# OpenVVC/VVCSoftware_VTM

Measured on AMD Instinct MI355X. Metric: encoded frames/sec (bit-exact bitstream) at 4K10 RA QP32, 1/2/4/8 GPU [M1: hot-path pictures/s of the kernels behind the call sites, NOT EncoderApp fps], higher is better.
Workload: dtype int16

## Files before the change

### vvcsoftware_vtm_amd/csrc/alf.hip

```cpp
#include "common.h"
#include <cstddef>

namespace {

constexpr int CT = 64;
constexpr int CP = 72;
constexpr int CR = CT + 6;
constexpr int QN = CT / 4 + 1;

template <int PITCH>
__device__ __forceinline__ void load_tile_clamped(short* __restrict__ lds, const Pel* __restrict__ src,
                                                  int stride, int w, int h, int x0, int y0, int rows,
                                                  int tid, int nthreads)
{
  constexpr int VPR = PITCH / 4;
  const int nvec = rows * VPR;
  const bool vec_ok = ((stride & 3) == 0) && ((reinterpret_cast<uintptr_t>(src) & 7) == 0);
  for (int v = tid; v < nvec; v += nthreads)
  {
    const int r = v / VPR, c = (v - r * VPR) * 4;
    int y = y0 + r;
    y = y < 0 ? 0 : (y >= h ? h - 1 : y);
    const int x = x0 + c;
    const Pel* row = src + (size_t)y * stride;
    pel4 val;
    if (vec_ok && x >= 0 && x + 3 < w)
      val = *reinterpret_cast<const pel4*>(row + x);
    else
    {
#pragma unroll
      for (int k = 0; k < 4; k++)
      {
        int xx = x + k;
        xx = xx < 0 ? 0 : (xx >= w ? w - 1 : xx);
        val[k] = row[xx];
      }
    }
    *reinterpret_cast<pel4*>(lds + r * PITCH + c) = val;
  }
}

__global__ __launch_bounds__(320) void alf_classify_kernel(const Pel* __restrict__ src, int stride, int w, int h,
                                                           int shift, uint16_t* __restrict__ cls, int gx, int total, int xcd)
{
  __shared__ short tile[CR * CP];
  __shared__ int quad[QN * QN * 4];
  const int tid = threadIdx.x;
  const int b = vvc_xcd_index((int)blockIdx.x, total, xcd);
  if (b < 0) return;
  const int by = b / gx, bx = b - by * gx;
  const int tx0 = bx * CT, ty0 = by * CT;
  load_tile_clamped<CP>(tile, src, stride, w, h, tx0 - 4, ty0 - 3, CR, tid, 320);
  __syncthreads();

  if (tid < QN * QN)
  {
    const int qi = tid / QN, qj = tid - qi * QN;
    const unsigned* base = reinterpret_cast<const unsigned*>(tile + (4 * qi) * CP + 4 * qj);
    unsigned sv = 0, sh = 0, sd0 = 0, sd1 = 0;
    unsigned A[5], B[5], C[5];
    auto loadRow = [&](int r, unsigned (&P)[5])
    {
      const uint2 lo = *reinterpret_cast<const uint2*>(base + r * (CP / 2)), hi = *reinterpret_cast<const uint2*>(base + r * (CP / 2) + 2);
      P[0] = __builtin_amdgcn_alignbit(lo.y, lo.x, 16); P[1] = lo.y; P[2] = __builtin_amdgcn_alignbit(hi.x, lo.y, 16); P[3] = hi.x;
      P[4] = __builtin_amdgcn_alignbit(hi.y, hi.x, 16);
    };
    typedef unsigned short us2v __attribute__((ext_vector_type(2)));
    auto padd = [](unsigned a, unsigned b) { return __builtin_bit_cast(unsigned, __builtin_bit_cast(us2v, a) + __builtin_bit_cast(us2v, b)); };
    loadRow(0, A); loadRow(1, B);
#pragma unroll
    for (int y = 0; y < 4; y++)
    {
      loadRow(y + 2, C);
      const unsigned c01 = padd(B[1], B[1]), c23 = padd(B[3], B[3]);
      sv  = __builtin_amdgcn_sad_u16(c01, padd(A[1], C[1]), sv);   sv  = __builtin_amdgcn_sad_u16(c23, padd(A[3], C[3]), sv);
      sh  = __builtin_amdgcn_sad_u16(c01, padd(B[0], B[2]), sh);   sh  = __builtin_amdgcn_sad_u16(c23, padd(B[2], B[4]), sh);
      sd0 = __builtin_amdgcn_sad_u16(c01, padd(A[0], C[2]), sd0);  sd0 = __builtin_amdgcn_sad_u16(c23, padd(A[2], C[4]), sd0);
      sd1 = __builtin_amdgcn_sad_u16(c01, padd(C[0], A[2]), sd1);  sd1 = __builtin_amdgcn_sad_u16(c23, padd(C[2], A[4]), sd1);
#pragma unroll
      for (int k = 0; k < 5; k++) { A[k] = B[k]; B[k] = C[k]; }
    }
    int* q = quad + tid * 4;
    q[0] = (int)sv; q[1] = (int)sh; q[2] = (int)sd0; q[3] = (int)sd1;
  }
  __syncthreads();

  if (tid < 256)
  {
    const int bi = tid >> 4, bj = tid & 15;
    const int by = ty0 + 4 * bi, bx = tx0 + 4 * bj;
    if (by < h && bx < w)
    {
      const int* q00 = quad + (bi * QN + bj) * 4;
      const int* q01 = q00 + 4;
      const int* q10 = q00 + QN * 4;
      const int* q11 = q10 + 4;
      const int sumV = q00[0] + q01[0] + q10[0] + q11[0];
      const int sumH = q00[1] + q01[1] + q10[1] + q11[1];
      const int sumD0 = q00[2] + q01[2] + q10[2] + q11[2];
      const int sumD1 = q00[3] + q01[3] + q10[3] + q11[3];
      const unsigned long long th = 0x4333333332222210ull;
      const int activity = (short)clip3(0, 15, ((sumV + sumH) * 32) >> shift);
      int classIdx = (int)((th >> (4 * activity)) & 15);
      int hv1, hv0, d1, d0, dirHV, dirD;
      if (sumV > sumH) { hv1 = sumV; hv0 = sumH; dirHV = 1; } else { hv1 = sumH; hv0 = sumV; dirHV = 3; }
      if (sumD0 > sumD1) { d1 = sumD0; d0 = sumD1; dirD = 0; } else { d1 = sumD1; d0 = sumD0; dirD = 2; }
      int hvd1, hvd0, mainDir, secDir;
      if ((int)((unsigned)d1 * (unsigned)hv0) > (int)((unsigned)hv1 * (unsigned)d0))
      { hvd1 = d1; hvd0 = d0; mainDir = dirD; secDir = dirHV; }
      else
      { hvd1 = hv1; hvd0 = hv0; mainDir = dirHV; secDir = dirD; }
      int strength = 0;
      if (hvd1 > 2 * hvd0) strength = 1;
      if (hvd1 * 2 > 9 * hvd0) strength = 2;
      if (strength) classIdx += (((mainDir & 1) << 1) + strength) * 5;
      const int transposeIdx = (0xDE84u >> (2 * (mainDir * 2 + (secDir >> 1)))) & 3;
      cls[(size_t)(by >> 2) * (w >> 2) + (bx >> 2)] = (uint16_t)(classIdx | (transposeIdx << 8));
    }
  }
}

constexpr int FW = 64, FH = 32;
constexpr int FP = FW + 8;
constexpr int FR = FH + 6;

struct AlfCoeffs { int16_t c[25 * 13]; };

template <bool IS7>
__device__ __forceinline__ constexpr int tapIndex(int dy, int dx)
{
  if (dy < 0 || (dy == 0 && dx < 0)) { dy = -dy; dx = -dx; }
  if (IS7)
  {
    if (dy == 3) return dx == 0 ? 0 : -1;
    if (dy == 2) return dx == 1 ? 1 : dx == 0 ? 2 : dx == -1 ? 3 : -1;
    if (dy == 1) return (dx >= -2 && dx <= 2) ? 6 - dx : -1;
    return dx <= 3 ? 12 - dx : -1;
  }
  else
  {
    if (dy == 2) return dx == 0 ? 0 : -1;
    if (dy == 1) return (dx >= -1 && dx <= 1) ? 2 - dx : -1;
    if (dy == 0) return dx <= 2 ? 6 - dx : -1;
    return -1;
  }
}

template <bool IS7, bool LUMA>
__device__ __forceinline__ void alf_filter_body(const int bidx, const int bidy, short* tile, short* scoef, const Pel* __restrict__ src, int sstride,
                                                         Pel* __restrict__ dst, int dstride, int w, int h,
                                                         int ctu, int wCtu, const uint16_t* __restrict__ cls,
                                                         const int16_t* __restrict__ coeffs, const uint8_t* __restrict__ ctuEnable,
                                                         int clpMin, int clpMax)
{
  const int tid = threadIdx.x;
  const int tx0 = bidx * FW, ty0 = bidy * FH;
  load_tile_clamped<FP>(tile, src, sstride, w, h, tx0 - 4, ty0 - 3, FR, tid, 128);
  for (int i = tid; i < (LUMA ? 25 * 13 : 7); i += 128) scoef[i] = coeffs[i];
  __syncthreads();

  const int bj = tid & 15, bi = tid >> 4;
  const int bx = tx0 + 4 * bj, by = ty0 + 4 * bi;
  if (bx >= w || by >= h) return;
  constexpr int R = IS7 ? 3 : 2;
  constexpr int NC = IS7 ? 13 : 7;
  const bool enabled = !ctuEnable || ctuEnable[(by / ctu) * wCtu + bx / ctu];
  const short* p = tile + (4 * bi + 3 - R) * FP + 4 * bj;

  if (!enabled)
  {
#pragma unroll
    for (int y = 0; y < 4; y++)
      *reinterpret_cast<pel4*>(dst + (size_t)(by + y) * dstride + bx) =
          *reinterpret_cast<const pel4*>(p + (R + y) * FP + 4);
    return;
  }

  int f[NC];
  if (LUMA)
  {
    const uint16_t c = cls[(size_t)(by >> 2) * (w >> 2) + (bx >> 2)];
    const short* cf = scoef + (c & 0xff) * 13;
    const int t = c >> 8;
    if (IS7)
    {
      const unsigned long long perm = t == 0 ? 0xCBA9876543210ull : t == 1 ? 0xC62037B518A49ull
                                    : t == 2 ? 0xCBA9456781230ull : 0xC62015B734A89ull;
#pragma unroll
      for (int i = 0; i < 13; i++) f[i] = cf[(perm >> (4 * i)) & 15];
    }
    else
    {
      const unsigned perm = t == 0 ? 0x6543210u : t == 1 ? 0x6203514u : t == 2 ? 0x6541230u : 0x6201534u;
#pragma unroll
      for (int i = 0; i < 7; i++) f[i] = cf[(perm >> (4 * i)) & 15];
    }
  }
  else
  {
#pragma unroll
    for (int i = 0; i < NC; i++) f[i] = scoef[i];
  }

  int acc[4][4];
#pragma unroll
  for (int i = 0; i < 4; i++)
#pragma unroll
    for (int j = 0; j < 4; j++) acc[i][j] = 0;

  typedef short s2v __attribute__((ext_vector_type(2)));
  unsigned cpk[2 * R + 1][R + 1];
#pragma unroll
  for (int dy = -R; dy <= R; dy++)
  {
    const int wid = R - (dy < 0 ? -dy : dy);
#pragma unroll
    for (int q = 0; q <= R; q++)
    {
      const int dx0 = -wid + 2 * q;
      unsigned v = 0;
      if (dx0 <= wid)
      {
        const int ka = tapIndex<IS7>(dy, dx0);
        v = (unsigned)f[ka] & 0xFFFFu;
        if (dx0 + 1 <= wid) v |= (unsigned)f[tapIndex<IS7>(dy, dx0 + 1)] << 16;
      }
      cpk[dy + R][q] = v;
    }
  }
#pragma unroll
  for (int r = 0; r < 4 + 2 * R; r++)
  {
    unsigned E[6], O[5];
    const uint2 v0 = *reinterpret_cast<const uint2*>(p + r * FP), v1 = *reinterpret_cast<const uint2*>(p + r * FP + 4), v2 = *reinterpret_cast<const uint2*>(p + r * FP + 8);
    E[0] = v0.x; E[1] = v0.y; E[2] = v1.x; E[3] = v1.y; E[4] = v2.x; E[5] = v2.y;
#pragma unroll
    for (int m = 0; m < 5; m++) O[m] = __builtin_amdgcn_alignbit(E[m + 1], E[m], 16);
#pragma unroll
    for (int i = 0; i < 4; i++)
    {
      const int dy = r - R - i;
      if (dy < -R || dy > R) continue;
      const int wid = R - (dy < 0 ? -dy : dy);
#pragma unroll
      for (int q = 0; q <= R; q++)
      {
        const int dx0 = -wid + 2 * q;
        if (dx0 > wid) continue;
        const s2v cp = __builtin_bit_cast(s2v, cpk[dy + R][q]);
#pragma unroll
        for (int j = 0; j < 4; j++)
        {
          const int idx = 4 + j + dx0;
          const unsigned sp = (idx & 1) ? O[(idx - 1) >> 1] : E[idx >> 1];
          acc[i][j] = __builtin_amdgcn_sdot2(__builtin_bit_cast(s2v, sp), cp, acc[i][j], false);
        }
      }
    }
  }
#pragma unroll
  for (int i = 0; i < 4; i++)
  {
    pel4 o;
#pragma unroll
    for (int j = 0; j < 4; j++) o[j] = (short)clip3(clpMin, clpMax, (acc[i][j] + 256) >> 9);
    *reinterpret_cast<pel4*>(dst + (size_t)(by + i) * dstride + bx) = o;
  }
}

__device__ __forceinline__ const int16_t* alf_kernarg(size_t off)
{
#if defined(__HIP_DEVICE_COMPILE__)
  return reinterpret_cast<const int16_t*>((const char*)__builtin_amdgcn_kernarg_segment_ptr() + off);
#else
  (void)off; return nullptr;
#endif
}
struct AlfFilterArgs { const Pel* src; int sstride; Pel* dst; int dstride, w, h, ctu, wCtu; const uint16_t* cls; AlfCoeffs coeffs; const uint8_t* ctuEnable; int clpMin, clpMax; };

template <bool IS7, bool LUMA>
__global__ __launch_bounds__(128) void alf_filter_kernel(AlfFilterArgs a)
{
  __shared__ short tile[FR * FP];
  __shared__ short scoef[25 * 13 + 3];
  alf_filter_body<IS7, LUMA>((int)blockIdx.x, (int)blockIdx.y, tile, scoef, a.src, a.sstride, a.dst, a.dstride, a.w, a.h, a.ctu, a.wCtu, a.cls,
                             alf_kernarg(offsetof(AlfFilterArgs, coeffs)), a.ctuEnable, a.clpMin, a.clpMax);
}

struct AlfPlane { const Pel* src; Pel* dst; const uint8_t* enable; int sstride, dstride; };
struct AlfFilter3 { AlfPlane a[3]; const uint16_t* cls; int w, h, ctu, glx, nLuma, gcx, gcy, clpMin, clpMax, total, xcd; AlfCoeffs luma; short chroma[8]; };
template <bool IS7>
__global__ __launch_bounds__(128) void alf_filter_picture_kernel(AlfFilter3 p)
{
  __shared__ short tile[FR * FP];
  __shared__ short scoef[25 * 13 + 3];
  const int b = vvc_xcd_index2((int)blockIdx.x, p.nLuma, p.total, p.xcd);
  if (b < 0) return;
  if (b < p.nLuma)
    alf_filter_body<IS7, true>(b % p.glx, b / p.glx, tile, scoef, p.a[0].src, p.a[0].sstride, p.a[0].dst, p.a[0].dstride, p.w, p.h, p.ctu, (p.w + p.ctu - 1) / p.ctu,
                               p.cls, alf_kernarg(offsetof(AlfFilter3, luma)), p.a[0].enable, p.clpMin, p.clpMax);
  else
  {
    const int c = b - p.nLuma, per = p.gcx * p.gcy, z = c / per, r = c - z * per;
    const AlfPlane& a = z ? p.a[2] : p.a[1];
    const int ctuC = p.ctu >> 1, wc = p.w >> 1;
    alf_filter_body<false, false>(r % p.gcx, r / p.gcx, tile, scoef, a.src, a.sstride, a.dst, a.dstride, wc, p.h >> 1, ctuC, (wc + ctuC - 1) / ctuC,
                                  nullptr, alf_kernarg(offsetof(AlfFilter3, chroma)), a.enable, p.clpMin, p.clpMax);
  }
}


}

extern "C" {

int vvcgpu_alf_classify(const vvc_pel* src, int src_stride, int width, int height, int bit_depth,
                        uint16_t* cls, void* stream)
{
  VVC_CHECK_ARG(src && cls, "alf_classify: null pointer");
  VVC_CHECK_ARG(width > 0 && height > 0 && (width & 3) == 0 && (height & 3) == 0,
                "alf_classify: width/height must be positive multiples of 4 (got %dx%d)", width, height);
  VVC_CHECK_ARG(src_stride >= width, "alf_classify: stride %d < width %d", src_stride, width);
  VVC_CHECK_ARG(bit_depth >= 8 && bit_depth <= 10, "alf_classify: bit depth %d outside 8..10", bit_depth);
  const int gx = cdiv(width, CT), total = gx * cdiv(height, CT), xcd = vvc_xcd_on();
  hipLaunchKernelGGL(alf_classify_kernel, dim3(vvc_xcd_grid(total, xcd)), dim3(320), 0, (hipStream_t)stream, src, src_stride, width, height,
                     bit_depth + 4, cls, gx, total, xcd);
  VVC_LAUNCH_CHECK();
  return VVCGPU_OK;
}

static int alf_filter_common(bool luma, const vvc_pel* src, int src_stride, vvc_pel* dst, int dst_stride,
                             int width, int height, int ctu_size, const uint16_t* cls, int filter_type,
                             const int16_t* coeff_host, const uint8_t* ctu_enable, int clp_min, int clp_max,
                             void* stream)
{
  VVC_CHECK_ARG(src && dst && coeff_host, "alf_filter: null pointer");
  VVC_CHECK_ARG(src != dst, "alf_filter: src must not alias dst");
  VVC_CHECK_ARG(!luma || cls, "alf_filter_luma: null classifier");
  VVC_CHECK_ARG(width > 0 && height > 0 && (width & 3) == 0 && (height & 3) == 0,
                "alf_filter: width/height must be positive multiples of 4 (got %dx%d)", width, height);
  VVC_CHECK_ARG(src_stride >= width && dst_stride >= width && (dst_stride & 3) == 0,
                "alf_filter: bad strides %d/%d (dst stride must be a multiple of 4)", src_stride, dst_stride);
  VVC_CHECK_ARG(((uintptr_t)dst & 7) == 0, "alf_filter: dst must be 8-byte aligned");
  VVC_CHECK_ARG(ctu_size >= 4 && (ctu_size & 3) == 0, "alf_filter: bad ctu size %d", ctu_size);
  VVC_CHECK_ARG(filter_type == 0 || filter_type == 1, "alf_filter: filter_type %d", filter_type);
  AlfCoeffs cf;
  memset(&cf, 0, sizeof cf);
  memcpy(cf.c, coeff_host, sizeof(int16_t) * (luma ? 25 * 13 : 7));
  dim3 grid(cdiv(width, FW), cdiv(height, FH));
  const int wCtu = cdiv(width, ctu_size);
  hipStream_t st = (hipStream_t)stream;
  AlfFilterArgs ka{ src, src_stride, dst, dst_stride, width, height, ctu_size, wCtu, cls, cf, ctu_enable, clp_min, clp_max };
  if (luma && filter_type == 1)
    hipLaunchKernelGGL((alf_filter_kernel<true, true>), grid, dim3(128), 0, st, ka);
  else if (luma)
    hipLaunchKernelGGL((alf_filter_kernel<false, true>), grid, dim3(128), 0, st, ka);
  else
    hipLaunchKernelGGL((alf_filter_kernel<false, false>), grid, dim3(128), 0, st, ka);
  VVC_LAUNCH_CHECK();
  return VVCGPU_OK;
}

int vvcgpu_alf_filter_luma(const vvc_pel* src, int src_stride, vvc_pel* dst, int dst_stride,
                           int width, int height, int ctu_size, const uint16_t* cls,
                           int filter_type, const int16_t* coeff_host, const uint8_t* ctu_enable,
                           int clp_min, int clp_max, void* stream)
{
  return alf_filter_common(true, src, src_stride, dst, dst_stride, width, height, ctu_size, cls, filter_type,
                           coeff_host, ctu_enable, clp_min, clp_max, stream);
}

int vvcgpu_alf_filter_chroma(const vvc_pel* src, int src_stride, vvc_pel* dst, int dst_stride,
                             int width, int height, int ctu_size, const int16_t* coeff_host,
                             const uint8_t* ctu_enable, int clp_min, int clp_max, void* stream)
{
  return alf_filter_common(false, src, src_stride, dst, dst_stride, width, height, ctu_size, nullptr, 0,
                           coeff_host, ctu_enable, clp_min, clp_max, stream);
}

int vvcgpu_alf_filter_picture(const vvcgpu_planes* src, const vvcgpu_planes* dst, int width, int height, int ctu_size, const uint16_t* cls,
                              int filter_type, const int16_t* luma_coeff_host, const int16_t* chroma_coeff_host, const uint8_t* enable_y,
                              const uint8_t* enable_cb, const uint8_t* enable_cr, int clp_min, int clp_max, void* stream)
{
  VVC_CHECK_ARG(src && dst && cls && luma_coeff_host && chroma_coeff_host, "alf_filter_picture: null pointer");
  VVC_CHECK_ARG(width > 0 && height > 0 && (width & 7) == 0 && (height & 7) == 0, "alf_filter_picture: width/height must be multiples of 8 (got %dx%d)", width, height);
  VVC_CHECK_ARG(ctu_size >= 8 && (ctu_size & 7) == 0, "alf_filter_picture: bad ctu size %d", ctu_size);
  VVC_CHECK_ARG(filter_type == 0 || filter_type == 1, "alf_filter_picture: filter_type %d", filter_type);
  AlfFilter3 p;
  memset(&p, 0, sizeof p);
  const uint8_t* en[3] = { enable_y, enable_cb, enable_cr };
  for (int c = 0; c < 3; c++)
  {
    const int w = c ? width >> 1 : width;
    VVC_CHECK_ARG(src->p[c] && dst->p[c] && src->p[c] != dst->p[c] && src->stride[c] >= w && dst->stride[c] >= w && (dst->stride[c] & 3) == 0 &&
                  ((uintptr_t)dst->p[c] & 7) == 0, "alf_filter_picture: plane %d (dst needs stride %% 4 == 0 and 8-byte alignment)", c);
    p.a[c] = AlfPlane{ src->p[c], dst->p[c], en[c], src->stride[c], dst->stride[c] };
  }
  memcpy(p.luma.c, luma_coeff_host, sizeof(int16_t) * 25 * 13);
  memcpy(p.chroma, chroma_coeff_host, sizeof(int16_t) * 7);
  p.cls = cls; p.w = width; p.h = height; p.ctu = ctu_size; p.clpMin = clp_min; p.clpMax = clp_max;
  p.glx = cdiv(width, FW); p.nLuma = p.glx * cdiv(height, FH);
  p.gcx = cdiv(width >> 1, FW); p.gcy = cdiv(height >> 1, FH);
  const int total = p.nLuma + 2 * p.gcx * p.gcy;
  p.total = total; p.xcd = vvc_xcd_on();
  if (filter_type) hipLaunchKernelGGL(alf_filter_picture_kernel<true>, dim3(vvc_xcd_grid2(p.nLuma, total, p.xcd)), dim3(128), 0, (hipStream_t)stream, p);
  else             hipLaunchKernelGGL(alf_filter_picture_kernel<false>, dim3(vvc_xcd_grid2(p.nLuma, total, p.xcd)), dim3(128), 0, (hipStream_t)stream, p);
  VVC_LAUNCH_CHECK();
  return VVCGPU_OK;
}

}
```

Before: 2063.

## Convert ALF filter to persistent XCD-chunked kernel with prefetched tiles and coefficient table

Replaces the one-workgroup-per-tile ALF launch with a persistent grid sized to resident occupancy. Each workgroup walks XCD-local chunks of luma and chroma tiles and prefetches the next tile's pixels and class/enable info into registers while filtering the current one. Per-class/transpose packed tap rows are built once into LDS, which removes the per-block coefficient permutation. It also adds magic-number division, med3 clipping, row-register prefetch and bias folding into the accumulator. The cost is more register pressure, extra complexity, and possible load imbalance from static chunking.

New measurement: 2055, median of 2. No clear change (-0.4%).

```diff
diff --git a/vvcsoftware_vtm_amd/csrc/alf.hip b/vvcsoftware_vtm_amd/csrc/alf.hip
--- a/vvcsoftware_vtm_amd/csrc/alf.hip
+++ b/vvcsoftware_vtm_amd/csrc/alf.hip
@@ -123,6 +123,10 @@
 constexpr int FW = 64, FH = 32;
 constexpr int FP = FW + 8;
 constexpr int FR = FH + 6;
+constexpr int FVPR = FP / 4;
+constexpr int FT = 128;
+constexpr int FNB = (FR * FVPR + FT - 1) / FT;
+static_assert(FT / FVPR * FVPR + 2 == FT && 2 * (FNB - 1) < FVPR, "alf_vec_pos: 128 = 7 rows of 18 vectors + 2");
 
 struct AlfCoeffs { int16_t c[25 * 13]; };
 
@@ -146,93 +150,104 @@
   }
 }
 
-template <bool IS7, bool LUMA>
-__device__ __forceinline__ void alf_filter_body(const int bidx, const int bidy, short* tile, short* scoef, const Pel* __restrict__ src, int sstride,
-                                                         Pel* __restrict__ dst, int dstride, int w, int h,
-                                                         int ctu, int wCtu, const uint16_t* __restrict__ cls,
-                                                         const int16_t* __restrict__ coeffs, const uint8_t* __restrict__ ctuEnable,
-                                                         int clpMin, int clpMax)
-{
-  const int tid = threadIdx.x;
-  const int tx0 = bidx * FW, ty0 = bidy * FH;
-  load_tile_clamped<FP>(tile, src, sstride, w, h, tx0 - 4, ty0 - 3, FR, tid, 128);
-  for (int i = tid; i < (LUMA ? 25 * 13 : 7); i += 128) scoef[i] = coeffs[i];
-  __syncthreads();
-
-  const int bj = tid & 15, bi = tid >> 4;
-  const int bx = tx0 + 4 * bj, by = ty0 + 4 * bi;
-  if (bx >= w || by >= h) return;
-  constexpr int R = IS7 ? 3 : 2;
-  constexpr int NC = IS7 ? 13 : 7;
-  const bool enabled = !ctuEnable || ctuEnable[(by / ctu) * wCtu + bx / ctu];
-  const short* p = tile + (4 * bi + 3 - R) * FP + 4 * bj;
-
-  if (!enabled)
-  {
-#pragma unroll
-    for (int y = 0; y < 4; y++)
-      *reinterpret_cast<pel4*>(dst + (size_t)(by + y) * dstride + bx) =
-          *reinterpret_cast<const pel4*>(p + (R + y) * FP + 4);
-    return;
-  }
-
-  int f[NC];
-  if (LUMA)
-  {
-    const uint16_t c = cls[(size_t)(by >> 2) * (w >> 2) + (bx >> 2)];
-    const short* cf = scoef + (c & 0xff) * 13;
-    const int t = c >> 8;
-    if (IS7)
-    {
-      const unsigned long long perm = t == 0 ? 0xCBA9876543210ull : t == 1 ? 0xC62037B518A49ull
-                                    : t == 2 ? 0xCBA9456781230ull : 0xC62015B734A89ull;
-#pragma unroll
-      for (int i = 0; i < 13; i++) f[i] = cf[(perm >> (4 * i)) & 15];
-    }
-    else
-    {
-      const unsigned perm = t == 0 ? 0x6543210u : t == 1 ? 0x6203514u : t == 2 ? 0x6541230u : 0x6201534u;
-#pragma unroll
-      for (int i = 0; i < 7; i++) f[i] = cf[(perm >> (4 * i)) & 15];
-    }
+template <bool IS7> struct AlfDiamond
+{
+  static constexpr int R = IS7 ? 3 : 2, NC = IS7 ? 13 : 7, NS = (R + 1) * (R + 1);
+  static constexpr int PITCH = IS7 ? 20 : 12;
+  static constexpr int NV = PITCH / 4;
+  static __device__ __forceinline__ constexpr int slot(int a, int q) { return (a <= R ? a * (a + 1) / 2 : NS - (2 * R + 1 - a) * (2 * R + 2 - a) / 2) + q; }
+};
+
+template <bool IS7>
+__device__ __forceinline__ void alf_pack_taps(const int (&f)[AlfDiamond<IS7>::NC], unsigned (&tv)[AlfDiamond<IS7>::PITCH])
+{
+  typedef AlfDiamond<IS7> D;
+  constexpr int R = D::R;
+#pragma unroll
+  for (int s = 0; s < D::PITCH; s++) tv[s] = 0;
+#pragma unroll
+  for (int dy = -R; dy <= R; dy++)
+  {
+    const int wid = R - (dy < 0 ? -dy : dy);
+#pragma unroll
+    for (int q = 0; q <= R; q++)
+    {
+      const int dx0 = -wid + 2 * q;
+      if (dx0 > wid) continue;
+      unsigned v = (unsigned)f[tapIndex<IS7>(dy, dx0)] & 0xFFFFu;
+      if (dx0 + 1 <= wid) v |= (unsigned)f[tapIndex<IS7>(dy, dx0 + 1)] << 16;
+      tv[D::slot(dy + R, q)] = v;
+    }
+  }
+}
+
+template <bool IS7>
+__device__ __forceinline__ void alf_luma_row(const int16_t* __restrict__ coeffs, int cls, int t, unsigned (&tv)[AlfDiamond<IS7>::PITCH])
+{
+  const int16_t* cf = coeffs + cls * 13;
+  int f[AlfDiamond<IS7>::NC];
+  if (IS7)
+  {
+    const unsigned long long perm = t == 0 ? 0xCBA9876543210ull : t == 1 ? 0xC62037B518A49ull
+                                  : t == 2 ? 0xCBA9456781230ull : 0xC62015B734A89ull;
+#pragma unroll
+    for (int i = 0; i < 13; i++) f[i] = cf[(perm >> (4 * i)) & 15];
   }
   else
   {
-#pragma unroll
-    for (int i = 0; i < NC; i++) f[i] = scoef[i];
-  }
-
+    const unsigned perm = t == 0 ? 0x6543210u : t == 1 ? 0x6203514u : t == 2 ? 0x6541230u : 0x6201534u;
+#pragma unroll
+    for (int i = 0; i < 7; i++) f[i] = cf[(perm >> (4 * i)) & 15];
+  }
+  alf_pack_taps<IS7>(f, tv);
+}
+
+#if defined(__HIP_DEVICE_COMPILE__)
+#define ALF_GLOBAL __attribute__((address_space(1)))
+#else
+#define ALF_GLOBAL
+#endif
+typedef const ALF_GLOBAL Pel* AlfSrc;
+#if defined(__HIP_DEVICE_COMPILE__)
+#define ALF_ROW_FENCE(a) asm volatile("" : "+v"(a[0][0]), "+v"(a[0][1]), "+v"(a[0][2]), "+v"(a[0][3]), "+v"(a[1][0]), "+v"(a[1][1]), "+v"(a[1][2]), "+v"(a[1][3]), \
+                                           "+v"(a[2][0]), "+v"(a[2][1]), "+v"(a[2][2]), "+v"(a[2][3]), "+v"(a[3][0]), "+v"(a[3][1]), "+v"(a[3][2]), "+v"(a[3][3]) :: "memory")
+#else
+#define ALF_ROW_FENCE(a)
+#endif
+
+__device__ __forceinline__ int alf_clip(int lo, int hi, int v)
+{
+#if defined(__HIP_DEVICE_COMPILE__)
+  int r;
+  asm("v_med3_i32 %0, %1, %2, %3" : "=v"(r) : "v"(v), "v"(lo), "v"(hi));
+  return r;
+#else
+  return v < lo ? lo : v > hi ? hi : v;
+#endif
+}
+
+template <bool IS7>
+__device__ __forceinline__ void alf_block(const short* __restrict__ p, const unsigned (&tv)[AlfDiamond<IS7>::PITCH], ALF_GLOBAL Pel* __restrict__ out, int dstride,
+                                          int clpMin, int clpMax)
+{
+  typedef AlfDiamond<IS7> D;
+  constexpr int R = D::R;
+  typedef short s2v __attribute__((ext_vector_type(2)));
   int acc[4][4];
 #pragma unroll
   for (int i = 0; i < 4; i++)
 #pragma unroll
-    for (int j = 0; j < 4; j++) acc[i][j] = 0;
-
-  typedef short s2v __attribute__((ext_vector_type(2)));
-  unsigned cpk[2 * R + 1][R + 1];
-#pragma unroll
-  for (int dy = -R; dy <= R; dy++)
-  {
-    const int wid = R - (dy < 0 ? -dy : dy);
-#pragma unroll
-    for (int q = 0; q <= R; q++)
-    {
-      const int dx0 = -wid + 2 * q;
-      unsigned v = 0;
-      if (dx0 <= wid)
-      {
-        const int ka = tapIndex<IS7>(dy, dx0);
-        v = (unsigned)f[ka] & 0xFFFFu;
-        if (dx0 + 1 <= wid) v |= (unsigned)f[tapIndex<IS7>(dy, dx0 + 1)] << 16;
-      }
-      cpk[dy + R][q] = v;
-    }
-  }
+    for (int j = 0; j < 4; j++) acc[i][j] = 256;
+  uint2 n0 = *reinterpret_cast<const uint2*>(p), n1 = *reinterpret_cast<const uint2*>(p + 4), n2 = *reinterpret_cast<const uint2*>(p + 8);
 #pragma unroll
   for (int r = 0; r < 4 + 2 * R; r++)
   {
     unsigned E[6], O[5];
-    const uint2 v0 = *reinterpret_cast<const uint2*>(p + r * FP), v1 = *reinterpret_cast<const uint2*>(p + r * FP + 4), v2 = *reinterpret_cast<const uint2*>(p + r * FP + 8);
+    const uint2 v0 = n0, v1 = n1, v2 = n2;
+    if (r + 1 < 4 + 2 * R)
+    {
+      n0 = *reinterpret_cast<const uint2*>(p + (r + 1) * FP); n1 = *reinterpret_cast<const uint2*>(p + (r + 1) * FP + 4); n2 = *reinterpret_cast<const uint2*>(p + (r + 1) * FP + 8);
+    }
     E[0] = v0.x; E[1] = v0.y; E[2] = v1.x; E[3] = v1.y; E[4] = v2.x; E[5] = v2.y;
 #pragma unroll
     for (int m = 0; m < 5; m++) O[m] = __builtin_amdgcn_alignbit(E[m + 1], E[m], 16);
@@ -247,7 +262,7 @@
       {
         const int dx0 = -wid + 2 * q;
         if (dx0 > wid) continue;
-        const s2v cp = __builtin_bit_cast(s2v, cpk[dy + R][q]);
+        const s2v cp = __builtin_bit_cast(s2v, tv[D::slot(dy + R, q)]);
 #pragma unroll
         for (int j = 0; j < 4; j++)
         {
@@ -257,14 +272,15 @@
         }
       }
     }
+    ALF_ROW_FENCE(acc);
   }
 #pragma unroll
   for (int i = 0; i < 4; i++)
   {
-    pel4 o;
-#pragma unroll
-    for (int j = 0; j < 4; j++) o[j] = (short)clip3(clpMin, clpMax, (acc[i][j] + 256) >> 9);
-    *reinterpret_cast<pel4*>(dst + (size_t)(by + i) * dstride + bx) = o;
+    unsigned o[4];
+#pragma unroll
+    for (int j = 0; j < 4; j++) o[j] = (unsigned)alf_clip(clpMin, clpMax, acc[i][j] >> 9);
+    *reinterpret_cast<ALF_GLOBAL uint2*>(out + (size_t)i * dstride) = make_uint2(__builtin_amdgcn_perm(o[1], o[0], 0x05040100u), __builtin_amdgcn_perm(o[3], o[2], 0x05040100u));
   }
 }
 
@@ -276,39 +292,195 @@
   (void)off; return nullptr;
 #endif
 }
-struct AlfFilterArgs { const Pel* src; int sstride; Pel* dst; int dstride, w, h, ctu, wCtu; const uint16_t* cls; AlfCoeffs coeffs; const uint8_t* ctuEnable; int clpMin, clpMax; };
-
-template <bool IS7, bool LUMA>
-__global__ __launch_bounds__(128) void alf_filter_kernel(AlfFilterArgs a)
-{
-  __shared__ short tile[FR * FP];
-  __shared__ short scoef[25 * 13 + 3];
-  alf_filter_body<IS7, LUMA>((int)blockIdx.x, (int)blockIdx.y, tile, scoef, a.src, a.sstride, a.dst, a.dstride, a.w, a.h, a.ctu, a.wCtu, a.cls,
-                             alf_kernarg(offsetof(AlfFilterArgs, coeffs)), a.ctuEnable, a.clpMin, a.clpMax);
-}
-
-struct AlfPlane { const Pel* src; Pel* dst; const uint8_t* enable; int sstride, dstride; };
-struct AlfFilter3 { AlfPlane a[3]; const uint16_t* cls; int w, h, ctu, glx, nLuma, gcx, gcy, clpMin, clpMax, total, xcd; AlfCoeffs luma; short chroma[8]; };
+
+__device__ __forceinline__ int alf_uniform(int v)
+{
+#if defined(__HIP_DEVICE_COMPILE__)
+  return __builtin_amdgcn_readfirstlane(v);
+#else
+  return v;
+#endif
+}
+
+__host__ __device__ __forceinline__ unsigned alf_div(unsigned x, unsigned d, unsigned magic)
+{
+#if defined(__HIP_DEVICE_COMPILE__)
+  return magic ? __umulhi(x, magic) : x / d;
+#else
+  return magic ? (unsigned)(((unsigned long long)x * magic) >> 32) : x / d;
+#endif
+}
+
+struct AlfPlane { const Pel* src; Pel* dst; const uint8_t* enable; int sstride, dstride, w, h, ctu, wCtu, gx, n, vec; unsigned ctuMagic, gxMagic; };
+struct AlfWalk { AlfPlane a[3]; const uint16_t* cls; int clpMin, clpMax, nx, chunkA, chunkC; short chroma[8]; AlfCoeffs luma; };
+
+struct AlfTile { AlfPlane pl; int tx0, ty0; bool luma; };
+
+__device__ __forceinline__ AlfPlane alf_walk_plane_arg(int pl)
+{
+  struct Bits { unsigned d[sizeof(AlfPlane) / 4]; } b;
+#if defined(__HIP_DEVICE_COMPILE__)
+  typedef const __attribute__((address_space(4))) char* kbytes;
+  typedef const __attribute__((address_space(4))) unsigned* kwords;
+  const kwords k = (kwords)((kbytes)__builtin_amdgcn_kernarg_segment_ptr() + offsetof(AlfWalk, a) + (size_t)pl * sizeof(AlfPlane));
+#pragma unroll
+  for (unsigned d = 0; d < sizeof(AlfPlane) / 4; d++) b.d[d] = k[d];
+#else
+  (void)pl; memset(&b, 0, sizeof b);
+#endif
+  return __builtin_bit_cast(AlfPlane, b);
+}
+
+__device__ __forceinline__ bool alf_vec_pos(int r0, int c0, int u, int& r, int& c)
+{
+  r = r0 + (FT / FVPR) * u; c = c0 + 2 * u;
+  if (c >= FVPR) { c -= FVPR; r++; }
+  return u < FNB - 1 || r < FR;
+}
+static_assert((FNB - 1) * FT <= FR * FVPR, "only a thread's last vector can be missing");
+
+__device__ __forceinline__ void alf_tile_fetch(pel4 (&pv)[FNB], const AlfTile& t, int r0, int c0)
+{
+  const AlfSrc src = (AlfSrc)t.pl.src;
+  const int stride = t.pl.sstride, w = t.pl.w, h = t.pl.h, x0 = t.tx0 - 4, y0 = t.ty0 - 3;
+  if (t.pl.vec && x0 >= 0 && x0 + FP <= w && y0 >= 0 && y0 + FR <= h)
+  {
+    const AlfSrc base = src + (size_t)y0 * stride + x0;
+#pragma unroll
+    for (int u = 0; u < FNB; u++)
+    {
+      int r, c;
+      pv[u] = pel4{ 0, 0, 0, 0 };
+      if (alf_vec_pos(r0, c0, u, r, c)) pv[u] = *reinterpret_cast<const ALF_GLOBAL pel4*>(base + r * stride + 4 * c);
+    }
+    return;
+  }
+#pragma unroll
+  for (int u = 0; u < FNB; u++)
+  {
+    int r, c;
+    pv[u] = pel4{ 0, 0, 0, 0 };
+    if (!alf_vec_pos(r0, c0, u, r, c)) continue;
+    int y = y0 + r;
+    y = y < 0 ? 0 : (y >= h ? h - 1 : y);
+    const int x = x0 + 4 * c;
+    const AlfSrc row = src + (size_t)y * stride;
+    if (t.pl.vec && x >= 0 && x + 3 < w) pv[u] = *reinterpret_cast<const ALF_GLOBAL pel4*>(row + x);
+    else
+    {
+#pragma unroll
+      for (int k = 0; k < 4; k++) { int xx = x + k; xx = xx < 0 ? 0 : (xx >= w ? w - 1 : xx); pv[u][k] = row[xx]; }
+    }
+  }
+}
+
 template <bool IS7>
-__global__ __launch_bounds__(128) void alf_filter_picture_kernel(AlfFilter3 p)
-{
-  __shared__ short tile[FR * FP];
-  __shared__ short scoef[25 * 13 + 3];
-  const int b = vvc_xcd_index2((int)blockIdx.x, p.nLuma, p.total, p.xcd);
-  if (b < 0) return;
-  if (b < p.nLuma)
-    alf_filter_body<IS7, true>(b % p.glx, b / p.glx, tile, scoef, p.a[0].src, p.a[0].sstride, p.a[0].dst, p.a[0].dstride, p.w, p.h, p.ctu, (p.w + p.ctu - 1) / p.ctu,
-                               p.cls, alf_kernarg(offsetof(AlfFilter3, luma)), p.a[0].enable, p.clpMin, p.clpMax);
-  else
-  {
-    const int c = b - p.nLuma, per = p.gcx * p.gcy, z = c / per, r = c - z * per;
-    const AlfPlane& a = z ? p.a[2] : p.a[1];
-    const int ctuC = p.ctu >> 1, wc = p.w >> 1;
-    alf_filter_body<false, false>(r % p.gcx, r / p.gcx, tile, scoef, a.src, a.sstride, a.dst, a.dstride, wc, p.h >> 1, ctuC, (wc + ctuC - 1) / ctuC,
-                                  nullptr, alf_kernarg(offsetof(AlfFilter3, chroma)), a.enable, p.clpMin, p.clpMax);
-  }
-}
-
+__global__ __launch_bounds__(FT) void alf_filter_picture_kernel(AlfWalk p)
+{
+  typedef AlfDiamond<IS7> D;
+  typedef AlfDiamond<false> DC;
+  __shared__ __attribute__((aligned(16))) short tile[FR * FP];
+  __shared__ __attribute__((aligned(16))) unsigned tab[100 * D::PITCH];
+  const int tid = threadIdx.x;
+  const int n0 = p.a[0].n, n1 = p.a[1].n, nC = n1 + p.a[2].n;
+  const bool x8 = p.nx == 8;
+  const int xcd = x8 ? (int)blockIdx.x & 7 : 0, nW = x8 ? (int)gridDim.x >> 3 : (int)gridDim.x;
+  const int firstA = xcd * p.chunkA, firstC = xcd * p.chunkC, len = p.chunkA + p.chunkC;
+  auto next = [&](int i) { while (i < len && !(i < p.chunkA ? firstA + i < n0 : firstC + i - p.chunkA < nC)) i += nW; return i; };
+  auto decode = [&](int i, AlfTile& t)
+  {
+    int b, pl = 0;
+    if (i < p.chunkA) b = firstA + i;
+    else { b = firstC + i - p.chunkA; pl = 1; if (b >= n1) { b -= n1; pl = 2; } }
+    b = alf_uniform(b); pl = alf_uniform(pl);
+    t.pl = alf_walk_plane_arg(pl);
+    const int ty = (int)alf_div((unsigned)b, (unsigned)t.pl.gx, t.pl.gxMagic);
+    t.tx0 = (b - ty * t.pl.gx) * FW; t.ty0 = ty * FH; t.luma = pl == 0;
+  };
+  int i = next(x8 ? (int)blockIdx.x >> 3 : (int)blockIdx.x);
+  if (i >= len) return;
+
+  unsigned tvc[DC::PITCH];
+  {
+    int f[DC::NC];
+#pragma unroll
+    for (int k = 0; k < DC::NC; k++) f[k] = p.chroma[k];
+    alf_pack_taps<false>(f, tvc);
+  }
+
+  const int r0 = tid / FVPR, c0 = tid - r0 * FVPR;
+  const int bj = tid & 15, bi = tid >> 4;
+  auto blockInfo = [&](const AlfTile& t, unsigned& c, unsigned& en)
+  {
+    const int bx = t.tx0 + 4 * bj, by = t.ty0 + 4 * bi;
+    c = 0; en = 1;
+    if (bx >= t.pl.w || by >= t.pl.h) return;
+    if (t.luma) c = p.cls[(size_t)(by >> 2) * (t.pl.w >> 2) + (bx >> 2)];
+    if (t.pl.enable) en = ((const ALF_GLOBAL uint8_t*)t.pl.enable)[alf_div((unsigned)by, (unsigned)t.pl.ctu, t.pl.ctuMagic) * t.pl.wCtu + alf_div((unsigned)bx, (unsigned)t.pl.ctu, t.pl.ctuMagic)];
+  };
+
+  pel4 pv[FNB];
+  unsigned ncls, nen;
+  {
+    AlfTile t;
+    decode(i, t);
+    alf_tile_fetch(pv, t, r0, c0);
+    blockInfo(t, ncls, nen);
+  }
+  if (n0 > 0 && tid < 100)
+  {
+    unsigned tv[D::PITCH];
+    alf_luma_row<IS7>(alf_kernarg(offsetof(AlfWalk, luma)), tid >> 2, tid & 3, tv);
+#pragma unroll
+    for (int k = 0; k < D::NV; k++) reinterpret_cast<uint4*>(tab + tid * D::PITCH)[k] = make_uint4(tv[4 * k], tv[4 * k + 1], tv[4 * k + 2], tv[4 * k + 3]);
+  }
+  for (;;)
+  {
+    const int icur = alf_uniform(i);
+    __syncthreads();
+#pragma unroll
+    for (int u = 0; u < FNB; u++)
+    {
+      int r, c;
+      if (alf_vec_pos(r0, c0, u, r, c)) *reinterpret_cast<pel4*>(tile + r * FP + 4 * c) = pv[u];
+    }
+    const unsigned c = ncls, en = nen;
+    __syncthreads();
+    i = alf_uniform(next(icur + nW));
+    if (i < len)
+    {
+      AlfTile t;
+      decode(i, t);
+      alf_tile_fetch(pv, t, r0, c0);
+      blockInfo(t, ncls, nen);
+    }
+
+    AlfTile cur;
+    decode(icur, cur);
+    const int bx = cur.tx0 + 4 * bj, by = cur.ty0 + 4 * bi;
+    if (bx < cur.pl.w && by < cur.pl.h)
+    {
+      ALF_GLOBAL Pel* out = (ALF_GLOBAL Pel*)cur.pl.dst + (size_t)by * cur.pl.dstride + bx;
+      if (!en)
+      {
+        const short* q = tile + (4 * bi + 3) * FP + 4 * bj + 4;
+#pragma unroll
+        for (int y = 0; y < 4; y++) *reinterpret_cast<ALF_GLOBAL pel4*>(out + (size_t)y * cur.pl.dstride) = *reinterpret_cast<const pel4*>(q + y * FP);
+      }
+      else if (cur.luma)
+      {
+        const uint4* row = reinterpret_cast<const uint4*>(tab + ((c & 0xff) * 4 + (c >> 8)) * D::PITCH);
+        unsigned tv[D::PITCH];
+#pragma unroll
+        for (int k = 0; k < D::NV; k++) { const uint4 v = row[k]; tv[4 * k] = v.x; tv[4 * k + 1] = v.y; tv[4 * k + 2] = v.z; tv[4 * k + 3] = v.w; }
+        alf_block<IS7>(tile + (4 * bi + 3 - D::R) * FP + 4 * bj, tv, out, cur.pl.dstride, p.clpMin, p.clpMax);
+      }
+      else
+        alf_block<false>(tile + (4 * bi + 3 - DC::R) * FP + 4 * bj, tvc, out, cur.pl.dstride, p.clpMin, p.clpMax);
+    }
+    if (i >= len) break;
+  }
+}
 
 }
 
@@ -329,6 +501,45 @@
   return VVCGPU_OK;
 }
 
+static unsigned alf_magic(unsigned d, unsigned xmax)
+{
+  return d >= 2 && (unsigned long long)xmax * d <= (1ull << 32) ? (unsigned)(((1ull << 32) + d - 1) / d) : 0u;
+}
+
+static void alf_walk_plane(AlfPlane& a, const Pel* src, int sstride, Pel* dst, int dstride, int w, int h, int ctu, const uint8_t* enable)
+{
+  a.src = src; a.dst = dst; a.enable = enable; a.sstride = sstride; a.dstride = dstride; a.w = w; a.h = h; a.ctu = ctu; a.wCtu = cdiv(w, ctu);
+  a.gx = cdiv(w, FW); a.n = a.gx * cdiv(h, FH);
+  a.vec = ((sstride & 3) == 0) && (((uintptr_t)src & 7) == 0);
+  a.ctuMagic = alf_magic((unsigned)ctu, (unsigned)(w > h ? w : h));
+  a.gxMagic = alf_magic((unsigned)a.gx, (unsigned)a.n);
+}
+
+static int alf_walk_launch(AlfWalk& p, int filter_type, int clp_min, int clp_max, hipStream_t st)
+{
+  p.clpMin = clp_min > clp_max ? clp_max : clp_min; p.clpMax = clp_max;
+  const void* kernel = filter_type ? reinterpret_cast<const void*>(alf_filter_picture_kernel<true>) : reinterpret_cast<const void*>(alf_filter_picture_kernel<false>);
+  static int resident[2] = { 0, 0 };
+  if (!resident[filter_type])
+  {
+    int nb = 0;
+    VVC_HIP(hipOccupancyMaxActiveBlocksPerMultiprocessor(&nb, kernel, FT, 0));
+    resident[filter_type] = nb > 0 ? nb : 1;
+  }
+  const int total = p.a[0].n + p.a[1].n + p.a[2].n;
+  int wgs = vvcgpu_cu_count() * resident[filter_type];
+  const char* wgsEnv = getenv("VVCGPU_ALF_WGS");
+  if (wgsEnv && atoi(wgsEnv) >= 1 && atoi(wgsEnv) < wgs) wgs = atoi(wgsEnv);
+  if (wgs >= 8) wgs &= ~7;
+  const int grid = min(wgs >= 8 ? cdiv(total, 8) * 8 : total, wgs);
+  p.nx = (grid & 7) == 0 ? 8 : 1;
+  p.chunkA = cdiv(p.a[0].n, p.nx); p.chunkC = cdiv(p.a[1].n + p.a[2].n, p.nx);
+  if (filter_type) hipLaunchKernelGGL(alf_filter_picture_kernel<true>, dim3(grid), dim3(FT), 0, st, p);
+  else             hipLaunchKernelGGL(alf_filter_picture_kernel<false>, dim3(grid), dim3(FT), 0, st, p);
+  VVC_LAUNCH_CHECK();
+  return VVCGPU_OK;
+}
+
 static int alf_filter_common(bool luma, const vvc_pel* src, int src_stride, vvc_pel* dst, int dst_stride,
                              int width, int height, int ctu_size, const uint16_t* cls, int filter_type,
                              const int16_t* coeff_host, const uint8_t* ctu_enable, int clp_min, int clp_max,
@@ -344,21 +555,13 @@
   VVC_CHECK_ARG(((uintptr_t)dst & 7) == 0, "alf_filter: dst must be 8-byte aligned");
   VVC_CHECK_ARG(ctu_size >= 4 && (ctu_size & 3) == 0, "alf_filter: bad ctu size %d", ctu_size);
   VVC_CHECK_ARG(filter_type == 0 || filter_type == 1, "alf_filter: filter_type %d", filter_type);
-  AlfCoeffs cf;
-  memset(&cf, 0, sizeof cf);
-  memcpy(cf.c, coeff_host, sizeof(int16_t) * (luma ? 25 * 13 : 7));
-  dim3 grid(cdiv(width, FW), cdiv(height, FH));
-  const int wCtu = cdiv(width, ctu_size);
-  hipStream_t st = (hipStream_t)stream;
-  AlfFilterArgs ka{ src, src_stride, dst, dst_stride, width, height, ctu_size, wCtu, cls, cf, ctu_enable, clp_min, clp_max };
-  if (luma && filter_type == 1)
-    hipLaunchKernelGGL((alf_filter_kernel<true, true>), grid, dim3(128), 0, st, ka);
-  else if (luma)
-    hipLaunchKernelGGL((alf_filter_kernel<false, true>), grid, dim3(128), 0, st, ka);
-  else
-    hipLaunchKernelGGL((alf_filter_kernel<false, false>), grid, dim3(128), 0, st, ka);
-  VVC_LAUNCH_CHECK();
-  return VVCGPU_OK;
+  AlfWalk p;
+  memset(&p, 0, sizeof p);
+  alf_walk_plane(p.a[luma ? 0 : 1], src, src_stride, dst, dst_stride, width, height, ctu_size, ctu_enable);
+  if (luma) memcpy(p.luma.c, coeff_host, sizeof(int16_t) * 25 * 13);
+  else      memcpy(p.chroma, coeff_host, sizeof(int16_t) * 7);
+  p.cls = cls;
+  return alf_walk_launch(p, luma ? filter_type : 0, clp_min, clp_max, (hipStream_t)stream);
 }
 
 int vvcgpu_alf_filter_luma(const vvc_pel* src, int src_stride, vvc_pel* dst, int dst_stride,
@@ -386,7 +589,7 @@
   VVC_CHECK_ARG(width > 0 && height > 0 && (width & 7) == 0 && (height & 7) == 0, "alf_filter_picture: width/height must be multiples of 8 (got %dx%d)", width, height);
   VVC_CHECK_ARG(ctu_size >= 8 && (ctu_size & 7) == 0, "alf_filter_picture: bad ctu size %d", ctu_size);
   VVC_CHECK_ARG(filter_type == 0 || filter_type == 1, "alf_filter_picture: filter_type %d", filter_type);
-  AlfFilter3 p;
+  AlfWalk p;
   memset(&p, 0, sizeof p);
   const uint8_t* en[3] = { enable_y, enable_cb, enable_cr };
   for (int c = 0; c < 3; c++)
@@ -394,19 +597,12 @@
     const int w = c ? width >> 1 : width;
     VVC_CHECK_ARG(src->p[c] && dst->p[c] && src->p[c] != dst->p[c] && src->stride[c] >= w && dst->stride[c] >= w && (dst->stride[c] & 3) == 0 &&
                   ((uintptr_t)dst->p[c] & 7) == 0, "alf_filter_picture: plane %d (dst needs stride %% 4 == 0 and 8-byte alignment)", c);
-    p.a[c] = AlfPlane{ src->p[c], dst->p[c], en[c], src->stride[c], dst->stride[c] };
+    alf_walk_plane(p.a[c], src->p[c], src->stride[c], dst->p[c], dst->stride[c], w, c ? height >> 1 : height, c ? ctu_size >> 1 : ctu_size, en[c]);
   }
   memcpy(p.luma.c, luma_coeff_host, sizeof(int16_t) * 25 * 13);
   memcpy(p.chroma, chroma_coeff_host, sizeof(int16_t) * 7);
-  p.cls = cls; p.w = width; p.h = height; p.ctu = ctu_size; p.clpMin = clp_min; p.clpMax = clp_max;
-  p.glx = cdiv(width, FW); p.nLuma = p.glx * cdiv(height, FH);
-  p.gcx = cdiv(width >> 1, FW); p.gcy = cdiv(height >> 1, FH);
-  const int total = p.nLuma + 2 * p.gcx * p.gcy;
-  p.total = total; p.xcd = vvc_xcd_on();
-  if (filter_type) hipLaunchKernelGGL(alf_filter_picture_kernel<true>, dim3(vvc_xcd_grid2(p.nLuma, total, p.xcd)), dim3(128), 0, (hipStream_t)stream, p);
-  else             hipLaunchKernelGGL(alf_filter_picture_kernel<false>, dim3(vvc_xcd_grid2(p.nLuma, total, p.xcd)), dim3(128), 0, (hipStream_t)stream, p);
-  VVC_LAUNCH_CHECK();
-  return VVCGPU_OK;
-}
-
-}
+  p.cls = cls;
+  return alf_walk_launch(p, filter_type, clp_min, clp_max, (hipStream_t)stream);
+}
+
+}
```
